# taohan10200/CRA5

Measured on AMD Instinct MI355X. Metric: ERA5 frames/s (721x1440x268) encode+decode, higher is better.
Workload: dtype f32 (3xf16-split MFMA, fp32 accumulate)

## Files before the change

cra5_amd/csrc/attention_split_f16.hip:

```cpp
#include <hip/hip_runtime.h>
#include <math.h>
#include <stdlib.h>

#include "../../include/cra5_amd.h"
#include "split.h"

CRA5_RANGE_TU(attn)

typedef float f32x16 __attribute__((ext_vector_type(16)));
typedef _Float16 half8 __attribute__((ext_vector_type(8)));
typedef _Float16 half4 __attribute__((ext_vector_type(4)));
typedef __fp16 fp16x4 __attribute__((__vector_size__(4 * sizeof(__fp16))));
#if defined(__HIP_DEVICE_COMPILE__)
#define CRA5_TR_READ(P) \
  __builtin_bit_cast(half4, __builtin_amdgcn_ds_read_tr16_b64_v4f16((__attribute__((address_space(3))) fp16x4 *)(P)))
#else
#define CRA5_TR_READ(P) (*reinterpret_cast<const half4 *>(P))
#endif

namespace {

__device__ __forceinline__ int xcd_remap(int bid, int nb) {
  const int q = nb / 8, r = nb % 8;
  const int xcd = bid % 8, within = bid / 8;
  const int base = (xcd < r) ? xcd * (q + 1) : r * (q + 1) + (xcd - r) * q;
  return base + within;
}

struct WinGeom {
  int H, W, wh, ww, nwc;
};

__device__ __forceinline__ int token_of(const WinGeom &g, int wr, int wc, int t) {
  if (g.ww == g.W && g.wh == g.H) return t;
  const int r = t / g.ww, c = t - r * g.ww;
  const int gr = wr * g.wh + r, gc = wc * g.ww + c;
  return (gr < g.H && gc < g.W) ? gr * g.W + gc : -1;
}

#ifdef CRA5_ATTN_TRACE
__device__ unsigned long long g_attn_trace[6 * 8192];
#define CRA5_ATRACE(SLOT, VAL)                                                                          \
  if (threadIdx.x == 0 && atrace_idx < 8192) g_attn_trace[atrace_idx * 6 + (SLOT)] = (VAL);
#else
#define CRA5_ATRACE(SLOT, VAL)
#endif

constexpr int HD = 64;
constexpr int KS = 72;
constexpr int VS = 96;
constexpr int MAX_WIN_TOKENS = 1152;

struct BalArgs {
  int groups;
  int n_full;
  int n_wg_pass;
  int rem_tile0;
  int rem;
  int n_grp;
  int nkt;
  int maxp;
  float *ws;
};
__host__ __device__ __forceinline__ long bal_cut(long S, int G, int c) { return S * c / G; }
__host__ __device__ __forceinline__ int bal_piece_of(long S, int G, long s) {
  int c = (int)(s * G / S);
  if (c > G - 1) c = G - 1;
  while (c > 0 && bal_cut(S, G, c) > s) --c;
  while (c < G - 1 && bal_cut(S, G, c + 1) <= s) ++c;
  return c;
}
constexpr int WS_ROW = 68;

template <int NW, bool HI, bool GLOBAL, bool BAL = false, bool PLAIN = false>
__global__ __launch_bounds__(NW * 64, (NW >= 8 ? 1 : (NW == 4 ? 3 : 2))) void window_attention_split_kernel(
    const unsigned short *__restrict__ qkv, long ldq ,
    const unsigned short *__restrict__ pad_row, float *__restrict__ out, unsigned short *__restrict__ out_s,
    int Kp_out, int C, int heads, WinGeom g, int q_tiles , float scale, BalArgs bal) {
  static_assert(!BAL || GLOBAL, "the balanced schedule is for whole-grid launches");
  static_assert(!PLAIN || HI, "plain rows carry no lo plane");
  constexpr int NT = NW * 64;
  constexpr int PPR = PLAIN ? 8 : 16;
  constexpr int PIECES = 32 * PPR;
  constexpr int STG = (PIECES + NT - 1) / NT;

  constexpr int KPL = 32 * KS + 32;
  constexpr int VPL = 32 * VS;
  constexpr int KBUF = 2 * KPL, VBUF = 2 * VPL;
  __shared__ __attribute__((aligned(16))) unsigned short lds[2 * KBUF + 2 * VBUF];
  unsigned short *Ks = lds;
  unsigned short *Vt = lds + 2 * KBUF;
  constexpr int TAB = GLOBAL ? 1 : MAX_WIN_TOKENS;
  __shared__ long long tab[TAB];

  const int L = g.wh * g.ww;
  int head, win, n_seg = 1;
  int seg_tile0[2] = {0, 0}, seg_nact[2] = {NW, NW}, seg_j0[2] = {0, 0}, seg_j1[2] = {L / 32, L / 32}, seg_part[2] = {-1, -1};
  int seg_grp[2] = {0, 0};
  if (BAL) {
    const int pass = blockIdx.x / bal.n_wg_pass, w = blockIdx.x - pass * bal.n_wg_pass;
    int slot;
    if ((heads & 7) == 0 && (bal.n_wg_pass & 7) == 0) {
      const int xcd = w & 7, s_ = w >> 3;
      head = xcd * (heads >> 3) + s_ / bal.groups;
      slot = s_ % bal.groups;
    } else {
      head = w / bal.groups;
      slot = w % bal.groups;
    }
    win = 0;
    if (pass < bal.n_full) {
      seg_tile0[0] = (pass * bal.groups + slot) * NW;
    } else {
      const long S = (long)bal.n_grp * bal.nkt;
      const long s0 = bal_cut(S, bal.groups, slot), s1 = bal_cut(S, bal.groups, slot + 1);
      n_seg = 0;
      for (long s = s0; s < s1;) {
        const int gq = (int)(s / bal.nkt);
        const long e = min(s1, (long)(gq + 1) * bal.nkt);
        if (n_seg < 2) {
          seg_grp[n_seg] = gq;
          seg_tile0[n_seg] = bal.rem_tile0 + gq * NW;
          seg_nact[n_seg] = min(NW, bal.rem - gq * NW);
          seg_j0[n_seg] = (int)(s - (long)gq * bal.nkt);
          seg_j1[n_seg] = (int)(e - (long)gq * bal.nkt);
          seg_part[n_seg] = slot - bal_piece_of(S, bal.groups, (long)gq * bal.nkt);
          ++n_seg;
        }
        s = e;
      }
    }
  } else {
    const int pid = xcd_remap(blockIdx.x, gridDim.x);
    const int qt = pid % q_tiles;
    const int wh_id = pid / q_tiles;
    head = wh_id % heads;
    win = wh_id / heads;
    seg_tile0[0] = qt * NW;
  }
  const int wr = win / g.nwc, wc = win - wr * g.nwc;

  const int tid = threadIdx.x, lane = tid & 63, wave = tid >> 6;
  const int l31 = lane & 31, h = lane >> 5;
  const int hoff = head * HD;
  const long qoff = (PLAIN ? 1L : 2L) * hoff, koff = (PLAIN ? 1L : 2L) * (C + hoff), voff = (PLAIN ? 1L : 2L) * (2 * C + hoff);

  if (!GLOBAL) {
    const long long pad_delta = reinterpret_cast<const char *>(pad_row) - reinterpret_cast<const char *>(qkv);
    for (int t = tid; t < L; t += NT) {
      const int tok = token_of(g, wr, wc, t);
      tab[t] = (tok >= 0) ? (long long)tok * ldq * 2 : pad_delta;
    }
  }
  constexpr bool IDLE_SKIP = !GLOBAL || BAL;
  bool tab_ready = GLOBAL;
#pragma unroll 1
  for (int seg = 0; seg < n_seg; ++seg) {
  const int tile0 = seg_tile0[seg], n_active = seg_nact[seg], j0 = seg_j0[seg], j1 = seg_j1[seg];
#ifdef CRA5_ATTN_TRACE
  const int atrace_idx = GLOBAL ? 8192 : (int)blockIdx.x;
  const unsigned long long atrace_c0 = clock64();
#endif
  CRA5_ATRACE(0, wall_clock64());
  const int tq = (tile0 + wave) * 32 + l31;
  const int q_tok = (tq < L && wave < n_active) ? token_of(g, wr, wc, tq) : -1;
  const bool wave_active = __any(q_tok >= 0);
  if (!__syncthreads_or(wave_active ? 1 : 0)) continue;
  tab_ready = true;

  half8 qh[4], ql[4];
  {
    const unsigned short *qrow = ((q_tok >= 0) ? qkv + (size_t)q_tok * ldq : pad_row) + qoff;
#pragma unroll
    for (int s = 0; s < 4; ++s) {
      const int chunk = s >> 1, pp = 2 * (s & 1) + h;
      if (PLAIN) {
        qh[s] = *reinterpret_cast<const half8 *>(qrow + 16 * s + 8 * h);
        ql[s] = qh[s];
      } else {
        qh[s] = *reinterpret_cast<const half8 *>(qrow + chunk * 64 + pp * 8);
        ql[s] = *reinterpret_cast<const half8 *>(qrow + chunk * 64 + 32 + pp * 8);
      }
    }
  }
  const float cexp = scale * 1.44269504088896340736f;
  f32x16 negm;
#pragma unroll
  for (int r = 0; r < 16; ++r) negm[r] = 0.f;
  if (HI) {
#pragma unroll
    for (int s = 0; s < 4; ++s)
#pragma unroll
      for (int e = 0; e < 8; ++e) qh[s][e] = (_Float16)((float)qh[s][e] * cexp);
  }
  const float cmax = HI ? 1.0f : cexp;

  f32x16 o[2];
#pragma unroll
  for (int t = 0; t < 2; ++t)
#pragma unroll
    for (int r = 0; r < 16; ++r) o[t][r] = 0.f;
  float m_run = HI ? 0.f : -INFINITY, l_run = 0.f;

  const int n_tiles = j1 - j0;
  uint4 sk0 = make_uint4(0u, 0u, 0u, 0u), sk1 = sk0, sv0 = sk0, sv1 = sk0;
  static_assert(STG == 1 || STG == 2, "staging below is written out for one or two 16-byte pieces per thread");
  constexpr bool TWO = STG == 2;
  const int krow0 = min(tid / PPR, 31), krow1 = min((tid + NT) / PPR, 31);
  const long kcol = koff + (tid % PPR) * 8;
  const long vcol = voff + (tid % PPR) * 8;
  const unsigned short *kq0 = qkv + (size_t)(krow0 + 32 * j0) * ldq + kcol;
  const unsigned short *kq1 = qkv + (size_t)(krow1 + 32 * j0) * ldq + kcol;
  const unsigned short *vq0 = qkv + (size_t)(krow0 + 32 * j0) * ldq + vcol;
  const unsigned short *vq1 = qkv + (size_t)(krow1 + 32 * j0) * ldq + vcol;
  const long tile_step = 32 * ldq;
#define CRA5_ROW(JJ, ROW) \
  reinterpret_cast<const unsigned short *>(reinterpret_cast<const char *>(qkv) + tab[(JJ)*32 + (ROW)])
  const bool stage0 = (NT <= PIECES) || (tid < PIECES);
  const bool stage1 = TWO && (tid + NT < PIECES);
#define CRA5_K_LOAD(J)                                                                    \
  if (stage0) {                                                                           \
    if (GLOBAL) {                                                                         \
      sk0 = *reinterpret_cast<const uint4 *>(kq0);                                        \
      if (stage1) sk1 = *reinterpret_cast<const uint4 *>(kq1);                            \
      const long st_ = ((J) < n_tiles - 1) ? tile_step : 0;  \
      kq0 += st_;                                                                         \
      kq1 += st_;                                                                         \
    } else {                                                                              \
      const int jj_ = min((J), n_tiles - 1);                                              \
      sk0 = *reinterpret_cast<const uint4 *>(CRA5_ROW(jj_, krow0) + kcol);                \
      if (stage1) sk1 = *reinterpret_cast<const uint4 *>(CRA5_ROW(jj_, krow1) + kcol);    \
    }                                                                                     \
  }
#define CRA5_V_LOAD(J)                                                                    \
  if (stage0) {                                                                           \
    if (GLOBAL) {                                                                         \
      sv0 = *reinterpret_cast<const uint4 *>(vq0);                                        \
      if (stage1) sv1 = *reinterpret_cast<const uint4 *>(vq1);                            \
      const long st_ = ((J) < n_tiles - 1) ? tile_step : 0;                               \
      vq0 += st_;                                                                         \
      vq1 += st_;                                                                         \
    } else {                                                                              \
      const int jj_ = min((J), n_tiles - 1);                                              \
      sv0 = *reinterpret_cast<const uint4 *>(CRA5_ROW(jj_, krow0) + vcol);                \
      if (stage1) sv1 = *reinterpret_cast<const uint4 *>(CRA5_ROW(jj_, krow1) + vcol);    \
    }                                                                                     \
  }
#define CRA5_K_STORE1(P, BUF)                                                             \
  {                                                                                       \
    const int idx = tid + (P)*NT;                                                         \
    if (idx < PIECES) {                                                                   \
      const int row = idx / PPR, piece = idx % PPR;                                       \
      const int plane = PLAIN ? 0 : (piece >> 2) & 1, d0 = PLAIN ? 8 * piece : 32 * (piece >> 3) + 8 * (piece & 3); \
      *reinterpret_cast<uint4 *>(Ks + (BUF)*KBUF + plane * KPL + row * KS + d0) = sk##P;  \
    }                                                                                     \
  }
#define CRA5_K_STORE(BUF) { CRA5_K_STORE1(0, BUF) if (TWO) CRA5_K_STORE1(1, BUF) }
#define CRA5_V_STORE1(P, BUF)                                                             \
  {                                                                                       \
    const int idx = tid + (P)*NT;                                                         \
    if (idx < PIECES) {                                                                   \
      const int row = idx / PPR, piece = idx % PPR;                                       \
      const int plane = PLAIN ? 0 : (piece >> 2) & 1, d0 = PLAIN ? 8 * piece : 32 * (piece >> 3) + 8 * (piece & 3); \
      *reinterpret_cast<uint4 *>(Vt + (BUF)*VBUF + plane * VPL + row * VS + d0) = sv##P;  \
    }                                                                                     \
  }
#define CRA5_V_STORE(BUF) { CRA5_V_STORE1(0, BUF) if (TWO) CRA5_V_STORE1(1, BUF) }
#define CRA5_SCORES(DST, KB)                                                              \
  {                                                                                       \
    f32x16 acc_;                                                                          \
    _Pragma("unroll") for (int r = 0; r < 16; ++r) acc_[r] = 0.f;                         \
    _Pragma("unroll") for (int st = 0; st < 4; ++st) {                                    \
      const half8 kh = *reinterpret_cast<const half8 *>(k_base + (KB)*KBUF + 16 * st);     \
      const half8 kl = *reinterpret_cast<const half8 *>(k_base + (KB)*KBUF + KPL + 16 * st); \
      if (!HI) {                                                                          \
        acc_ = __builtin_amdgcn_mfma_f32_32x32x16_f16(kl, qh[st], acc_, 0, 0, 0);         \
        acc_ = __builtin_amdgcn_mfma_f32_32x32x16_f16(kh, ql[st], acc_, 0, 0, 0);         \
      }                                                                                   \
      if (HI && st == 0) {                                                                \
        CRA5_MFMA_FROM(acc_, kh, qh[0], negm);                                            \
      } else {                                                                            \
        acc_ = __builtin_amdgcn_mfma_f32_32x32x16_f16(kh, qh[st], acc_, 0, 0, 0);         \
      }                                                                                   \
    }                                                                                     \
    DST = acc_;                                                                           \
  }
#if defined(__HIP_DEVICE_COMPILE__)
#define CRA5_MFMA_FROM(D, A, B, C) \
  asm("s_nop 3\n\tv_mfma_f32_32x32x16_f16 %0, %1, %2, %3" : "=&v"(D) : "v"(A), "v"(B), "v"(C))
#else
#define CRA5_MFMA_FROM(D, A, B, C) (D) = (C)
#endif

  const unsigned short *k_base = Ks + l31 * KS + 8 * h;
  const unsigned short *v_base = Vt + (4 * h + ((lane & 15) >> 2)) * VS + 16 * ((lane >> 4) & 1) + 4 * (lane & 3);

#if defined(__HIP_DEVICE_COMPILE__)
#define CRA5_XHALF_MAX(X)                                                                 \
  ({                                                                                      \
    float a_ = (X), b_ = (X), r_;                                                         \
    asm("s_nop 1\n\tv_permlane32_swap_b32_e32 %0, %1\n\ts_nop 1\n\tv_max_f32_e32 %2, %0, %1" \
        : "+v"(a_), "+v"(b_), "=v"(r_));                                                  \
    r_;                                                                                   \
  })
#define CRA5_MAX2_VALU(A, B)                                                              \
  ({                                                                                      \
    float r_;                                                                             \
    asm("v_max_f32_e32 %0, %1, %2" : "=v"(r_) : "v"(A), "v"(B));                          \
    r_;                                                                                   \
  })
#else
#define CRA5_XHALF_MAX(X) (X)
#define CRA5_MAX2_VALU(A, B) fmaxf((A), (B))
#endif
#if !defined(__HIP_DEVICE_COMPILE__)
#define CRA5_TILE_MAX(S)                                                                  \
  ({                                                                                      \
    float m_ = fmaxf(fmaxf(fmaxf(S[0], S[1]), fmaxf(S[2], S[3])), fmaxf(fmaxf(S[4], S[5]), fmaxf(S[6], S[7]))); \
    float n_ = fmaxf(fmaxf(fmaxf(S[8], S[9]), fmaxf(S[10], S[11])), fmaxf(fmaxf(S[12], S[13]), fmaxf(S[14], S[15]))); \
    CRA5_XHALF_MAX(fmaxf(m_, n_)) * cmax;       \
  })
#else
#define CRA5_MAX3(A, B, C) fmaxf(fmaxf((A), (B)), (C))
#define CRA5_TILE_MAX(S)                                                                  \
  ({                                                                                      \
    const float a_ = CRA5_MAX3(S[0], S[1], S[2]), b_ = CRA5_MAX3(S[3], S[4], S[5]), c_ = CRA5_MAX3(S[6], S[7], S[8]); \
    const float d_ = CRA5_MAX3(S[9], S[10], S[11]), e_ = CRA5_MAX3(S[12], S[13], S[14]);     \
    const float f_ = CRA5_MAX3(a_, b_, c_), g_ = CRA5_MAX3(d_, e_, S[15]);                   \
    CRA5_XHALF_MAX(CRA5_MAX2_VALU(f_, g_)) * cmax;  \
  })
#endif

  f32x16 s_cur;
  CRA5_K_LOAD(0);
  CRA5_V_LOAD(0);
  CRA5_K_STORE(0);
  CRA5_V_STORE(0);
  CRA5_K_LOAD(1);
  CRA5_K_STORE(1);
  __syncthreads();
  CRA5_K_LOAD(2);
  CRA5_V_LOAD(1);
  CRA5_SCORES(s_cur, 0);
  float mloc = CRA5_TILE_MAX(s_cur);
  __syncthreads();

  auto key_tile = [&](const int j, f32x16 &s_cur, f32x16 &s_next) __attribute__((always_inline)) {
    const int kb = (j + 1) & 1, vb = j & 1;
    if (!IDLE_SKIP || wave_active) {
    constexpr float DEFER_LOG2 = 8.0f;
    auto shift = [&](float delta, const bool rescale, f32x16 *also) __attribute__((always_inline)) {
      delta = (float)(_Float16)fminf(fmaxf(delta, -60000.f), 60000.f);
      if (rescale) {
        const float alpha = __builtin_amdgcn_exp2f(-delta);
        l_run *= alpha;
#pragma unroll
        for (int t = 0; t < 2; ++t)
#pragma unroll
          for (int r = 0; r < 16; ++r) o[t][r] *= alpha;
      }
      m_run += delta;
      half8 e0, bd;
#pragma unroll
      for (int e = 0; e < 8; ++e) {
        e0[e] = (_Float16)0.0f;
        bd[e] = (_Float16)0.0f;
      }
      e0[0] = (_Float16)(h == 0 ? 1.0f : 0.0f);
      bd[0] = (_Float16)(h == 0 ? -delta : 0.0f);
      s_cur = __builtin_amdgcn_mfma_f32_32x32x16_f16(e0, bd, s_cur, 0, 0, 0);
      negm = __builtin_amdgcn_mfma_f32_32x32x16_f16(e0, bd, negm, 0, 0, 0);
      if (also) *also = __builtin_amdgcn_mfma_f32_32x32x16_f16(e0, bd, *also, 0, 0, 0);
#if defined(__HIP_DEVICE_COMPILE__)
      asm volatile("s_nop 15\n\ts_nop 3" ::: "memory");
#endif
    };
    if (HI) {
      if (j == 0) shift(mloc, false, nullptr);
    } else if (!__all(mloc - m_run <= DEFER_LOG2)) {
      const float m_new = fmaxf(m_run, mloc);
      const float alpha = __builtin_amdgcn_exp2f(m_run - m_new);
      l_run *= alpha;
#pragma unroll
      for (int t = 0; t < 2; ++t)
#pragma unroll
        for (int r = 0; r < 16; ++r) o[t][r] *= alpha;
      m_run = m_new;
    }
    const float m_new = m_run;
    CRA5_SCORES(s_next, kb);
    float psum = 0.f;
    half8 ph[2], pl[2];
#if defined(__HIP_DEVICE_COMPILE__)
    if (HI) {
      typedef _Float16 half2v __attribute__((ext_vector_type(2)));
      typedef _Float16 half8v __attribute__((ext_vector_type(8)));
      const half2v ones = {(_Float16)1.0f, (_Float16)1.0f};
      auto exps = [&]() __attribute__((always_inline)) {
        psum = 0.f;
#pragma unroll
        for (int t = 0; t < 2; ++t) {
          half2v hp[4];
#pragma unroll
          for (int i = 0; i < 4; ++i) {
            hp[i] = half2v{(_Float16)__builtin_amdgcn_exp2f(s_cur[8 * t + 2 * i]), (_Float16)__builtin_amdgcn_exp2f(s_cur[8 * t + 2 * i + 1])};
            psum = __builtin_amdgcn_fdot2(hp[i], ones, psum, false);
          }
          ph[t] = half8v{hp[0][0], hp[0][1], hp[1][0], hp[1][1], hp[2][0], hp[2][1], hp[3][0], hp[3][1]};
        }
      };
      exps();
      constexpr float P_SAFE = 8192.0f;
      if (!__all(psum <= P_SAFE)) {
        const float mrel = CRA5_TILE_MAX(s_cur);
        shift(fmaxf(mrel, 0.f), true, &s_next);
        exps();
      }
#pragma unroll
      for (int t = 0; t < 2; ++t)
#pragma unroll
        for (int e = 0; e < 8; ++e) pl[t][e] = (_Float16)0.0f;
    } else
    {
      typedef _Float16 half2v __attribute__((ext_vector_type(2)));
#pragma unroll
      for (int r = 0; r < 16; r += 2) {
        const float p0 = __builtin_amdgcn_exp2f(fmaf(s_cur[r], cexp, -m_new));
        const float p1 = __builtin_amdgcn_exp2f(fmaf(s_cur[r + 1], cexp, -m_new));
        psum += p0;
        psum += p1;
        const half2v h2 = {(_Float16)p0, (_Float16)p1};
        const unsigned hh = __builtin_bit_cast(unsigned, h2);
        float d0, d1;
        asm("s_nop 0\n\tv_fma_mix_f32 %0, %2, -1.0, %3 op_sel_hi:[1,0,0]\n\t"
            "v_fma_mix_f32 %1, %2, -1.0, %4 op_sel:[1,0,0] op_sel_hi:[1,0,0]"
            : "=&v"(d0), "=&v"(d1) : "v"(hh), "v"(p0), "v"(p1));
        ph[r >> 3][r & 7] = h2[0];
        ph[r >> 3][(r & 7) + 1] = h2[1];
        pl[r >> 3][r & 7] = (_Float16)d0;
        pl[r >> 3][(r & 7) + 1] = (_Float16)d1;
      }
    }
#else
#pragma unroll
    for (int r = 0; r < 16; ++r) {
      const float p = HI ? (float)(_Float16)__builtin_amdgcn_exp2f(s_cur[r]) : __builtin_amdgcn_exp2f(fmaf(s_cur[r], cexp, -m_new));
      psum += p;
      const _Float16 hi = (_Float16)p;
      const _Float16 lo = (_Float16)(p - (float)hi);
      ph[r >> 3][r & 7] = hi;
      pl[r >> 3][r & 7] = lo;
    }
#endif
    l_run += psum;
#pragma unroll
    for (int t = 0; t < 2; ++t) {
      half8 vh[2], vl[2];
#pragma unroll
      for (int dt = 0; dt < 2; ++dt) {
        const unsigned short *vp = v_base + vb * VBUF + 16 * t * VS + 32 * dt;
        const unsigned short *vq = vp + VPL;
        const half4 a0 = CRA5_TR_READ(vp);
        const half4 a1 = CRA5_TR_READ(vp + 8 * VS);
        const half4 b0 = CRA5_TR_READ(vq);
        const half4 b1 = CRA5_TR_READ(vq + 8 * VS);
        vh[dt] = __builtin_shufflevector(a0, a1, 0, 1, 2, 3, 4, 5, 6, 7);
        vl[dt] = __builtin_shufflevector(b0, b1, 0, 1, 2, 3, 4, 5, 6, 7);
      }
      if (!HI) {
        o[0] = __builtin_amdgcn_mfma_f32_32x32x16_f16(vl[0], ph[t], o[0], 0, 0, 0);
        o[1] = __builtin_amdgcn_mfma_f32_32x32x16_f16(vl[1], ph[t], o[1], 0, 0, 0);
        o[0] = __builtin_amdgcn_mfma_f32_32x32x16_f16(vh[0], pl[t], o[0], 0, 0, 0);
        o[1] = __builtin_amdgcn_mfma_f32_32x32x16_f16(vh[1], pl[t], o[1], 0, 0, 0);
      }
      o[0] = __builtin_amdgcn_mfma_f32_32x32x16_f16(vh[0], ph[t], o[0], 0, 0, 0);
      o[1] = __builtin_amdgcn_mfma_f32_32x32x16_f16(vh[1], ph[t], o[1], 0, 0, 0);
    }
    if (!HI) mloc = CRA5_TILE_MAX(s_next);
    }
    CRA5_K_STORE(j & 1);
    CRA5_V_STORE((j + 1) & 1);
    CRA5_K_LOAD(j + 3);
    CRA5_V_LOAD(j + 2);
    __syncthreads();
  };
  CRA5_ATRACE(1, wall_clock64());
  f32x16 s_alt;
  const int n_loop = n_tiles;
  int jt = 0;
  for (; jt + 1 < n_loop; jt += 2) {
    key_tile(jt, s_cur, s_alt);
    key_tile(jt + 1, s_alt, s_cur);
  }
  if (jt < n_loop) key_tile(jt, s_cur, s_alt);
  CRA5_ATRACE(2, wall_clock64());
  CRA5_ATRACE(4, (unsigned long long)n_tiles);

  const float l_tot = l_run + __shfl_xor(l_run, 32, 64);
  if (BAL && seg_part[seg] >= 0) {
    if (q_tok >= 0) {
      float *wrow = bal.ws + (((((size_t)head * bal.n_grp + seg_grp[seg]) * bal.maxp + seg_part[seg]) * NW + wave) * 32 + l31) * WS_ROW;
#pragma unroll
      for (int t = 0; t < 2; ++t)
#pragma unroll
        for (int gq = 0; gq < 4; ++gq) {
          const int d = 32 * t + 8 * gq + 4 * h;
          *reinterpret_cast<float4 *>(wrow + d) = make_float4(o[t][4 * gq + 0], o[t][4 * gq + 1], o[t][4 * gq + 2], o[t][4 * gq + 3]);
        }
      if (h == 0) {
        wrow[64] = m_run;
        wrow[65] = l_tot;
      }
    }
    continue;
  }
  {
    const bool live = q_tok >= 0;
    const float inv = live ? 1.0f / l_tot : 0.0f;
    float *orow = (out && live) ? out + (size_t)q_tok * C + hoff : nullptr;
    unsigned short *srow = (out_s && live) ? out_s + (size_t)q_tok * 2 * Kp_out : nullptr;
#pragma unroll
    for (int t = 0; t < 2; ++t)
#pragma unroll
      for (int pr = 0; pr < 2; ++pr) {
        float va[4], vb[4];
#pragma unroll
        for (int k = 0; k < 4; ++k) {
          va[k] = o[t][4 * (2 * pr) + k] * inv;
          vb[k] = o[t][4 * (2 * pr + 1) + k] * inv;
        }
        if (orow) {
          *reinterpret_cast<float4 *>(orow + 32 * t + 16 * pr + 4 * h) = make_float4(va[0], va[1], va[2], va[3]);
          *reinterpret_cast<float4 *>(orow + 32 * t + 16 * pr + 8 + 4 * h) = make_float4(vb[0], vb[1], vb[2], vb[3]);
        }
        if (out_s) {
          unsigned ha0, la0, ha1, la1, hb0, lb0, hb1, lb1;
          cra5_split_pair(va[0], va[1], ha0, la0);
          cra5_split_pair(va[2], va[3], ha1, la1);
          cra5_split_pair(vb[0], vb[1], hb0, lb0);
          cra5_split_pair(vb[2], vb[3], hb1, lb1);
#if defined(__HIP_DEVICE_COMPILE__)
#define CRA5_SWAP32(A, B)                                                  \
  {                                                                        \
    const auto r_ = __builtin_amdgcn_permlane32_swap((A), (B), false, false); \
    (A) = r_[0];                                                           \
    (B) = r_[1];                                                           \
  }
          CRA5_SWAP32(ha0, hb0);
          CRA5_SWAP32(ha1, hb1);
          CRA5_SWAP32(la0, lb0);
          CRA5_SWAP32(la1, lb1);
#undef CRA5_SWAP32
#endif
          if (srow) {
            const int c0 = hoff + 32 * t + 16 * pr + 8 * h;
            unsigned short *sp = srow + (PLAIN ? c0 : (c0 >> 5) * 64 + (c0 & 31));
            *reinterpret_cast<uint4 *>(sp) = make_uint4(ha0, ha1, hb0, hb1);
            if (!HI) *reinterpret_cast<uint4 *>(sp + 32) = make_uint4(la0, la1, lb0, lb1);
          }
        }
      }
  }
  CRA5_ATRACE(3, wall_clock64());
  CRA5_ATRACE(5, clock64() - atrace_c0);
  }
  (void)tab_ready;
}

__global__ __launch_bounds__(256) void attention_merge_kernel(const float *__restrict__ ws, float *__restrict__ out,
                                                              unsigned short *__restrict__ out_s, int Kp_out, int C,
                                                              BalArgs bal, int nw, int plain) {
  const int t = blockIdx.x % nw, hg = blockIdx.x / nw;
  const int grp = hg % bal.n_grp, head = hg / bal.n_grp;
  if (grp * nw + t >= bal.rem) return;
  const long S = (long)bal.n_grp * bal.nkt;
  const int c0 = bal_piece_of(S, bal.groups, (long)grp * bal.nkt);
  const int c1 = bal_piece_of(S, bal.groups, (long)(grp + 1) * bal.nkt - 1);
  const int np = c1 - c0 + 1;
  const int q = threadIdx.x >> 3, d0 = (threadIdx.x & 7) * 8;
  const size_t pstride = (size_t)nw * 32 * WS_ROW;
  const float *base = ws + ((((size_t)head * bal.n_grp + grp) * bal.maxp) * nw + t) * 32 * WS_ROW + (size_t)q * WS_ROW;
  float M = -INFINITY;
  for (int c = 0; c < np; ++c) M = fmaxf(M, base[c * pstride + 64]);
  float acc[8] = {0.f, 0.f, 0.f, 0.f, 0.f, 0.f, 0.f, 0.f}, lsum = 0.f;
  for (int c = 0; c < np; ++c) {
    const float *r = base + c * pstride;
    const float a = __builtin_amdgcn_exp2f(r[64] - M);
    lsum = fmaf(r[65], a, lsum);
    const float4 v0 = *reinterpret_cast<const float4 *>(r + d0), v1 = *reinterpret_cast<const float4 *>(r + d0 + 4);
    acc[0] = fmaf(v0.x, a, acc[0]);
    acc[1] = fmaf(v0.y, a, acc[1]);
    acc[2] = fmaf(v0.z, a, acc[2]);
    acc[3] = fmaf(v0.w, a, acc[3]);
    acc[4] = fmaf(v1.x, a, acc[4]);
    acc[5] = fmaf(v1.y, a, acc[5]);
    acc[6] = fmaf(v1.z, a, acc[6]);
    acc[7] = fmaf(v1.w, a, acc[7]);
  }
  const float inv = 1.0f / lsum;
  const int tok = (bal.rem_tile0 + grp * nw + t) * 32 + q, col = head * HD + d0;
#pragma unroll
  for (int k = 0; k < 8; ++k) acc[k] *= inv;
  if (out) {
    *reinterpret_cast<float4 *>(out + (size_t)tok * C + col) = make_float4(acc[0], acc[1], acc[2], acc[3]);
    *reinterpret_cast<float4 *>(out + (size_t)tok * C + col + 4) = make_float4(acc[4], acc[5], acc[6], acc[7]);
  }
  if (out_s) {
    unsigned short *srow = out_s + (size_t)tok * 2 * Kp_out;
    if (plain) {
      cra5_store_plain4(srow, col, acc[0], acc[1], acc[2], acc[3]);
      cra5_store_plain4(srow, col + 4, acc[4], acc[5], acc[6], acc[7]);
    } else {
      cra5_store_split4(srow, col, acc[0], acc[1], acc[2], acc[3]);
      cra5_store_split4(srow, col + 4, acc[4], acc[5], acc[6], acc[7]);
    }
  }
}

int cu_count() {
  static const int n = [] {
    int dev = 0, v = 0;
    if (hipGetDevice(&dev) != hipSuccess) return 256;
    if (hipDeviceGetAttribute(&v, hipDeviceAttributeMultiprocessorCount, dev) != hipSuccess || v <= 0) return 256;
    return v;
  }();
  return n;
}

constexpr int NW_GLOBAL = 12;

bool balanced_plan(int L, int heads, BalArgs &b) {
  const int P = cu_count(), T = L / 32;
  if (P % heads) return false;
  b.groups = P / heads;
  b.n_full = T / (b.groups * NW_GLOBAL);
  b.rem_tile0 = b.n_full * b.groups * NW_GLOBAL;
  b.rem = T - b.rem_tile0;
  b.n_grp = (b.rem + NW_GLOBAL - 1) / NW_GLOBAL;
  b.nkt = T;
  b.n_wg_pass = heads * b.groups;
  b.ws = nullptr;
  b.maxp = 0;
  const long S = (long)b.n_grp * b.nkt;
  for (int g = 0; g < b.n_grp; ++g) {
    const int np = bal_piece_of(S, b.groups, (long)(g + 1) * b.nkt - 1) - bal_piece_of(S, b.groups, (long)g * b.nkt) + 1;
    if (np > b.maxp) b.maxp = np;
  }
  if (!(b.n_full >= 1 && (b.rem == 0 || (b.n_grp <= b.groups && S >= b.groups)))) return false;
  for (int c = 0; b.rem && c < b.groups; ++c) {
    const long s0 = bal_cut(S, b.groups, c), s1 = bal_cut(S, b.groups, c + 1);
    if (s1 > s0 && (s1 - 1) / b.nkt - s0 / b.nkt + 1 > 2) return false;
  }
  return true;
}

size_t balanced_ws_bytes(const BalArgs &b, int heads) {
  return (size_t)heads * b.n_grp * b.maxp * NW_GLOBAL * 32 * WS_ROW * sizeof(float);
}

template <bool HI, bool PLAIN = false>
int launch_balanced(const unsigned short *qkv, long ldq, const unsigned short *pad_row, float *out, unsigned short *out_s,
                    int Kp_out, int C, int heads, int H, int W, float scale, BalArgs b, float *ws, hipStream_t st) {
  WinGeom g;
  g.H = H;
  g.W = W;
  g.wh = H;
  g.ww = W;
  g.nwc = 1;
  b.ws = ws;
  const int n_pass = b.n_full + (b.rem ? 1 : 0);
  hipLaunchKernelGGL((window_attention_split_kernel<NW_GLOBAL, HI, true, true, PLAIN>), dim3(n_pass * b.n_wg_pass),
                     dim3(NW_GLOBAL * 64), 0, st, qkv, ldq, pad_row, out, out_s, Kp_out, C, heads, g, 0, scale, b);
  int rc = (int)hipGetLastError();
  if (rc || b.rem == 0) return rc;
  hipLaunchKernelGGL(attention_merge_kernel, dim3(heads * b.n_grp * NW_GLOBAL), dim3(256), 0, st, ws, out, out_s, Kp_out,
                     C, b, NW_GLOBAL, PLAIN ? 1 : 0);
  return (int)hipGetLastError();
}

template <int NW, bool HI, bool GLOBAL, bool PLAIN = false>
int launch(const unsigned short *qkv, long ldq, const unsigned short *pad_row, float *out, unsigned short *out_s,
           int Kp_out, int C, int heads, int H, int W, int wh, int ww, float scale, hipStream_t st) {
  WinGeom g;
  g.H = H;
  g.W = W;
  g.wh = wh;
  g.ww = ww;
  const int nwr = (H + wh - 1) / wh;
  g.nwc = (W + ww - 1) / ww;
  const int L = wh * ww;
  const int q_tiles = (L + NW * 32 - 1) / (NW * 32);
  hipLaunchKernelGGL((window_attention_split_kernel<NW, HI, GLOBAL, false, PLAIN>), dim3(q_tiles * nwr * g.nwc * heads), dim3(NW * 64), 0, st,
                     qkv, ldq, pad_row, out, out_s, Kp_out, C, heads, g, q_tiles, scale, BalArgs{});
  return (int)hipGetLastError();
}

}

static int attention_dispatch(const uint16_t *qkv_split, int qkv_kp, const uint16_t *pad_row_split, float *out,
                              uint16_t *out_split, int out_kp, int C, int heads, int H, int W, int wh, int ww,
                              float scale, int hi_only, void *workspace, size_t workspace_bytes, void *stream,
                              bool want_balanced) {
  if (!qkv_split || !pad_row_split || (!out && !out_split) || heads <= 0 || C % heads) return CRA5_ERR_ARG;
  if (C / heads != 64 || qkv_kp != 3 * C) return CRA5_ERR_ARG;
  if (wh <= 0 || ww <= 0 || H <= 0 || W <= 0 || (wh * ww) % 32) return CRA5_ERR_ARG;
  if (out_split && (out_kp < C || out_kp % 32)) return CRA5_ERR_ARG;
  if (((uintptr_t)qkv_split & 15) || ((uintptr_t)pad_row_split & 15)) return CRA5_ERR_ARG;
  hipStream_t st = (hipStream_t)stream;
  const int L = wh * ww;
  if (hi_only != 0 && hi_only != 1 && hi_only != 3) return CRA5_ERR_ARG;
  const bool plain = hi_only == 3;
  const long ldq = 2L * qkv_kp;
  const bool whole = (wh == H && ww == W);
  if (!whole && L > MAX_WIN_TOKENS) return CRA5_ERR_ARG;
#define CRA5_ATT_GO(NWV, HIV, GLV) \
  return launch<NWV, HIV, GLV>(qkv_split, ldq, pad_row_split, out, out_split, out_kp, C, heads, H, W, wh, ww, scale, st)
  if (whole) {
    BalArgs b;
    if (want_balanced && balanced_plan(L, heads, b) &&
        (balanced_ws_bytes(b, heads) == 0 ||
         (workspace && ((uintptr_t)workspace & 15) == 0 && workspace_bytes >= balanced_ws_bytes(b, heads)))) {
      float *ws = reinterpret_cast<float *>(workspace);
      if (plain)
        return launch_balanced<true, true>(qkv_split, ldq, pad_row_split, out, out_split, out_kp, C, heads, H, W, scale, b, ws, st);
      if (hi_only)
        return launch_balanced<true>(qkv_split, ldq, pad_row_split, out, out_split, out_kp, C, heads, H, W, scale, b, ws, st);
      return launch_balanced<false>(qkv_split, ldq, pad_row_split, out, out_split, out_kp, C, heads, H, W, scale, b, ws, st);
    }
    if (plain) return launch<NW_GLOBAL, true, true, true>(qkv_split, ldq, pad_row_split, out, out_split, out_kp, C, heads, H, W, wh, ww, scale, st);
    if (hi_only) CRA5_ATT_GO(NW_GLOBAL, true, true);
    CRA5_ATT_GO(NW_GLOBAL, false, true);
  }
  if (plain) return launch<4, true, false, true>(qkv_split, ldq, pad_row_split, out, out_split, out_kp, C, heads, H, W, wh, ww, scale, st);
  if (hi_only) CRA5_ATT_GO(4, true, false);
  CRA5_ATT_GO(4, false, false);
#undef CRA5_ATT_GO
}

#ifdef CRA5_ATTN_TRACE
extern "C" int cra5_debug_attn_trace(unsigned long long *host, int n_rows) {
  if (n_rows < 1 || n_rows > 8192) return CRA5_ERR_ARG;
  if (hipDeviceSynchronize() != hipSuccess) return CRA5_ERR_ARG;
  int rc = (int)hipMemcpyFromSymbol(host, HIP_SYMBOL(g_attn_trace), sizeof(unsigned long long) * 6 * n_rows);
  void *p = nullptr;
  if (hipGetSymbolAddress(&p, HIP_SYMBOL(g_attn_trace)) == hipSuccess) hipMemset(p, 0, sizeof(unsigned long long) * 6 * 8192);
  return rc;
}
#endif

extern "C" int cra5_window_attention_split(const uint16_t *qkv_split, int qkv_kp, const uint16_t *pad_row_split,
                                           float *out, uint16_t *out_split, int out_kp, int C, int heads, int H,
                                           int W, int wh, int ww, float scale, int hi_only, void *stream) {
  return attention_dispatch(qkv_split, qkv_kp, pad_row_split, out, out_split, out_kp, C, heads, H, W, wh, ww, scale,
                            hi_only, nullptr, 0, stream, false);
}

extern "C" size_t cra5_attention_workspace_bytes(int n_tokens, int heads) {
  BalArgs b;
  if (n_tokens <= 0 || heads <= 0 || (n_tokens % 32) || !balanced_plan(n_tokens, heads, b)) return 0;
  return balanced_ws_bytes(b, heads);
}

extern "C" int cra5_window_attention_split_ws(const uint16_t *qkv_split, int qkv_kp, const uint16_t *pad_row_split,
                                              float *out, uint16_t *out_split, int out_kp, int C, int heads, int H,
                                              int W, int wh, int ww, float scale, int hi_only, void *workspace,
                                              size_t workspace_bytes, void *stream) {
  return attention_dispatch(qkv_split, qkv_kp, pad_row_split, out, out_split, out_kp, C, heads, H, W, wh, ww, scale,
                            hi_only, workspace, workspace_bytes, stream, true);
}

extern "C" int cra5_attention_balanced_plan(int n_tokens, int heads, size_t *workspace_bytes) {
  BalArgs b;
  if (workspace_bytes) *workspace_bytes = 0;
  if (n_tokens <= 0 || heads <= 0 || (n_tokens % 32) || !balanced_plan(n_tokens, heads, b)) return 0;
  if (workspace_bytes) *workspace_bytes = balanced_ws_bytes(b, heads);
  return 1;
}
```

Measured before the change: 31.61.

## Hand-interleave QK and PV MFMAs with softmax exp/split in non-HI attention path

For the non-HI (full 3xf16 split) attention path, the per-key-tile body is restructured into an explicit software-pipelined schedule. The QK score MFMAs for the next tile and the PV MFMAs are interleaved with exp2, hi/lo split, V transpose reads and the tile-max reduction, with sched_barrier fences pinning the order. The goal is to hide VALU/transcendental latency and LDS reads behind MFMA execution instead of running them in separate phases. The cost is a rigid manual schedule that blocks compiler reordering, may raise register pressure, and drops the s_nop padding on the split asm.

```diff
diff --git a/cra5_amd/csrc/attention_split_f16.hip b/cra5_amd/csrc/attention_split_f16.hip
--- a/cra5_amd/csrc/attention_split_f16.hip
+++ b/cra5_amd/csrc/attention_split_f16.hip
@@ -388,6 +388,120 @@
       m_run = m_new;
     }
     const float m_new = m_run;
+#if defined(__HIP_DEVICE_COMPILE__)
+    if (!HI) {
+#define CRA5_FENCE() __builtin_amdgcn_sched_barrier(0)
+#define CRA5_STAGE(MFMA_STMT) \
+  CRA5_FENCE();               \
+  MFMA_STMT;                  \
+  CRA5_FENCE();
+#define CRA5_KFRAG(PLANE, ST) (*reinterpret_cast<const half8 *>(k_base + kb * KBUF + (PLANE)*KPL + 16 * (ST)))
+#define CRA5_MM(A, B, C) __builtin_amdgcn_mfma_f32_32x32x16_f16((A), (B), (C), 0, 0, 0)
+      typedef _Float16 half2v __attribute__((ext_vector_type(2)));
+      typedef unsigned u32x4 __attribute__((ext_vector_type(4)));
+      float p[16], psum = 0.f;
+      u32x4 phw[2], plw[2];
+      auto exp_half = [&](const int u) __attribute__((always_inline)) {
+        p[2 * u] = __builtin_amdgcn_exp2f(fmaf(s_cur[2 * u], cexp, -m_new));
+        p[2 * u + 1] = __builtin_amdgcn_exp2f(fmaf(s_cur[2 * u + 1], cexp, -m_new));
+      };
+      auto split_half = [&](const int u) __attribute__((always_inline)) {
+        const int r = 2 * u;
+        const half2v h2 = {(_Float16)p[r], (_Float16)p[r + 1]};
+        const unsigned hh = __builtin_bit_cast(unsigned, h2);
+        float d0, d1;
+        asm("v_fma_mix_f32 %0, %2, -1.0, %3 op_sel_hi:[1,0,0]\n\t"
+            "v_fma_mix_f32 %1, %2, -1.0, %4 op_sel:[1,0,0] op_sel_hi:[1,0,0]"
+            : "=&v"(d0), "=&v"(d1) : "v"(hh), "v"(p[r]), "v"(p[r + 1]));
+        psum += p[r];
+        psum += p[r + 1];
+        const half2v l2 = {(_Float16)d0, (_Float16)d1};
+        unsigned ll = __builtin_bit_cast(unsigned, l2);
+        asm("" : "+v"(ll));
+        phw[u >> 2][u & 3] = hh;
+        plw[u >> 2][u & 3] = ll;
+      };
+#define ph(T) __builtin_bit_cast(half8, phw[T])
+#define pl(T) __builtin_bit_cast(half8, plw[T])
+      half8 vh[2], vl[2];
+      auto v_frag = [&](const int t, const int plane, const int dt) __attribute__((always_inline)) {
+        const unsigned short *vp = v_base + vb * VBUF + plane * VPL + 16 * t * VS + 32 * dt;
+        const half4 a0 = CRA5_TR_READ(vp);
+        const half4 a1 = CRA5_TR_READ(vp + 8 * VS);
+        return __builtin_shufflevector(a0, a1, 0, 1, 2, 3, 4, 5, 6, 7);
+      };
+      half8 kh0 = CRA5_KFRAG(0, 0), kl0 = CRA5_KFRAG(1, 0), kh1 = CRA5_KFRAG(0, 1), kl1 = CRA5_KFRAG(1, 1);
+      f32x16 acc;
+#pragma unroll
+      for (int r = 0; r < 16; ++r) acc[r] = 0.f;
+      CRA5_STAGE(acc = CRA5_MM(kl0, qh[0], acc))
+      exp_half(0);
+      CRA5_STAGE(acc = CRA5_MM(kh0, ql[0], acc))
+      exp_half(1);
+      CRA5_STAGE(acc = CRA5_MM(kh0, qh[0], acc))
+      split_half(0);
+      const half8 kh2 = CRA5_KFRAG(0, 2), kl2 = CRA5_KFRAG(1, 2);
+      CRA5_STAGE(acc = CRA5_MM(kl1, qh[1], acc))
+      exp_half(2);
+      CRA5_STAGE(acc = CRA5_MM(kh1, ql[1], acc))
+      split_half(1);
+      CRA5_STAGE(acc = CRA5_MM(kh1, qh[1], acc))
+      exp_half(3);
+      const half8 kh3 = CRA5_KFRAG(0, 3), kl3 = CRA5_KFRAG(1, 3);
+      CRA5_STAGE(acc = CRA5_MM(kl2, qh[2], acc))
+      split_half(2);
+      CRA5_STAGE(acc = CRA5_MM(kh2, ql[2], acc))
+      exp_half(4);
+      CRA5_STAGE(acc = CRA5_MM(kh2, qh[2], acc))
+      split_half(3);
+      CRA5_STAGE(acc = CRA5_MM(kl3, qh[3], acc))
+      exp_half(5);
+      vl[0] = v_frag(0, 1, 0);
+      vl[1] = v_frag(0, 1, 1);
+      CRA5_STAGE(acc = CRA5_MM(kh3, ql[3], acc))
+      split_half(4);
+      CRA5_STAGE(acc = CRA5_MM(kh3, qh[3], acc))
+      split_half(5);
+      vh[0] = v_frag(0, 0, 0);
+      vh[1] = v_frag(0, 0, 1);
+      s_next = acc;
+      CRA5_STAGE(o[0] = CRA5_MM(vl[0], ph(0), o[0]))
+      exp_half(6);
+      CRA5_STAGE(o[1] = CRA5_MM(vl[1], ph(0), o[1]))
+      exp_half(7);
+      CRA5_STAGE(o[0] = CRA5_MM(vh[0], pl(0), o[0]))
+      split_half(6);
+      CRA5_STAGE(o[1] = CRA5_MM(vh[1], pl(0), o[1]))
+      split_half(7);
+      vl[0] = v_frag(1, 1, 0);
+      vl[1] = v_frag(1, 1, 1);
+      CRA5_STAGE(o[0] = CRA5_MM(vh[0], ph(0), o[0]))
+      l_run += psum;
+      CRA5_STAGE(o[1] = CRA5_MM(vh[1], ph(0), o[1]))
+      vh[0] = v_frag(1, 0, 0);
+      vh[1] = v_frag(1, 0, 1);
+      CRA5_STAGE(o[0] = CRA5_MM(vl[0], ph(1), o[0]))
+      const float ma = CRA5_MAX3(s_next[0], s_next[1], s_next[2]), mb = CRA5_MAX3(s_next[3], s_next[4], s_next[5]);
+      const float mc = CRA5_MAX3(s_next[6], s_next[7], s_next[8]), md = CRA5_MAX3(s_next[9], s_next[10], s_next[11]);
+      const float me = CRA5_MAX3(s_next[12], s_next[13], s_next[14]);
+      CRA5_STAGE(o[1] = CRA5_MM(vl[1], ph(1), o[1]))
+      const float mf = CRA5_MAX3(ma, mb, mc), mg = CRA5_MAX3(md, me, s_next[15]);
+      const float mfg = CRA5_MAX2_VALU(mf, mg);
+      CRA5_STAGE(o[0] = CRA5_MM(vh[0], pl(1), o[0]))
+      const float mx = CRA5_XHALF_MAX(mfg);
+      CRA5_STAGE(o[1] = CRA5_MM(vh[1], pl(1), o[1]))
+      mloc = mx * cmax;
+      CRA5_STAGE(o[0] = CRA5_MM(vh[0], ph(1), o[0]))
+      CRA5_STAGE(o[1] = CRA5_MM(vh[1], ph(1), o[1]))
+#undef ph
+#undef pl
+#undef CRA5_MM
+#undef CRA5_KFRAG
+#undef CRA5_STAGE
+#undef CRA5_FENCE
+    } else
+#endif
+    {
     CRA5_SCORES(s_next, kb);
     float psum = 0.f;
     half8 ph[2], pl[2];
@@ -420,26 +534,6 @@
       for (int t = 0; t < 2; ++t)
 #pragma unroll
         for (int e = 0; e < 8; ++e) pl[t][e] = (_Float16)0.0f;
-    } else
-    {
-      typedef _Float16 half2v __attribute__((ext_vector_type(2)));
-#pragma unroll
-      for (int r = 0; r < 16; r += 2) {
-        const float p0 = __builtin_amdgcn_exp2f(fmaf(s_cur[r], cexp, -m_new));
-        const float p1 = __builtin_amdgcn_exp2f(fmaf(s_cur[r + 1], cexp, -m_new));
-        psum += p0;
-        psum += p1;
-        const half2v h2 = {(_Float16)p0, (_Float16)p1};
-        const unsigned hh = __builtin_bit_cast(unsigned, h2);
-        float d0, d1;
-        asm("s_nop 0\n\tv_fma_mix_f32 %0, %2, -1.0, %3 op_sel_hi:[1,0,0]\n\t"
-            "v_fma_mix_f32 %1, %2, -1.0, %4 op_sel:[1,0,0] op_sel_hi:[1,0,0]"
-            : "=&v"(d0), "=&v"(d1) : "v"(hh), "v"(p0), "v"(p1));
-        ph[r >> 3][r & 7] = h2[0];
-        ph[r >> 3][(r & 7) + 1] = h2[1];
-        pl[r >> 3][r & 7] = (_Float16)d0;
-        pl[r >> 3][(r & 7) + 1] = (_Float16)d1;
-      }
     }
 #else
 #pragma unroll
@@ -477,6 +571,7 @@
       o[1] = __builtin_amdgcn_mfma_f32_32x32x16_f16(vh[1], ph[t], o[1], 0, 0, 0);
     }
     if (!HI) mloc = CRA5_TILE_MAX(s_next);
+    }
     }
     CRA5_K_STORE(j & 1);
     CRA5_V_STORE((j + 1) & 1);
```

Measured after the change: 32.02 (median of 6 runs). 1.3% higher.
